# MDIL-SNU/SevenNet

Measured on NVIDIA H100. Metric: atom_updates_per_sec, higher is better.
Workload: dtype f32

## Files before the change

sevenn_b200/csrc/engine.cu:

```cuda
#include <algorithm>
#include <cstdlib>
#include <cstring>
#include <functional>
#include <map>
#include <string>
#include <vector>

#include "../../include/sevenn_b200.h"
#include "common.cuh"
#include "conv_kernels.cuh"
#include "edge_kernels.cuh"
#include "neighbor.cuh"
#include "node_kernels.cuh"
#include "tc_gemm.cuh"

namespace s7b {

static thread_local std::string g_error;
static int64_t g_launches = 0;
extern int64_t g_conv_launches;

void set_error(const char* file, int line, const char* msg) {
  char buf[512];
  snprintf(buf, sizeof(buf), "%s:%d: %s", file, line, msg);
// ... 329 lines not shown
  for (int n = 0; n < N; ++n) {
    double amax = 0.0;
    for (int k = 0; k < K; ++k) amax = std::max(amax, (double)fabsf(W[(size_t)k * N + n]));
    int Eb = 0;
    const bool zero = !(amax > 1e-30);
    if (!zero) frexp(amax, &Eb);
    fb[n] = zero ? 0.0f : (float)ldexp(1.0, Eb - 7);
    const int nt = n / NT, r = n % NT;
    for (int k = 0; k < K; ++k) {
      double sl[3] = {0.0, 0.0, 0.0};
      if (!zero) {
        const double t = ldexp((double)W[(size_t)k * N + n], 23 - Eb);
        const double q0 = nearbyint(t / 65536.0);
        const double r1 = t - q0 * 65536.0;
        const double q1 = nearbyint(r1 / 256.0);
        const double r2 = r1 - q1 * 256.0;
        const double q2 = nearbyint(r2);
        sl[0] = q0; sl[1] = q1 / 256.0; sl[2] = q2 / 65536.0;
      }
      const int kc = k / kTcKC, kk = k % kTcKC;
      const size_t elem = (size_t)((r & 7) * 16 + (r >> 3) * 512 + (kk >> 3) * 128 + (kk & 7) * 2) / 2;
      for (int sidx = 0; sidx < 3; ++sidx)
        q[(((size_t)nt * n_kc + kc) * 3 + sidx) * ((size_t)NT * kTcKC) + elem] = bf16_bits_exact((float)sl[sidx]);
    }
  }
}

static int tc_build_weights(TcWeights& w, const float* host, const int* Ks, const int* Ns, int n_l) {
  w.ok = false;
  w.nblocks = 0;
  size_t q_total = 0, fb_total = 0, woff = 0;
  for (int l = 0; l < n_l; ++l) {
    const int K = Ks[l], N = Ns[l];
    if (K == 0 || N == 0) continue;
    const int NT = tc_pick_nt(N);
    if (NT == 0 || K % kTcKC != 0) return 0;
    TcWeights::Blk& b = w.blk[w.nblocks++];
    b = {K, N, NT, q_total, fb_total};
    q_total += (size_t)3 * K * NT * tc_tiles(N, NT);
    fb_total += (size_t)N;
  }
  std::vector<uint16_t> q(q_total);
  std::vector<float> fb(fb_total);
  int bi = 0;
  for (int l = 0; l < n_l; ++l) {
    const int K = Ks[l], N = Ns[l];
    if (K == 0 || N == 0) continue;
    const TcWeights::Blk& b = w.blk[bi++];
    tc_pack_block(host + woff, K, N, b.NT, q.data() + b.q_off, fb.data() + b.fb_off);
    woff += (size_t)K * N;
  }
  if (w.q.ensure(q_total * sizeof(uint16_t) + 16) || w.fb.ensure(fb_total * sizeof(float) + 16)) return fail("cudaMalloc failed for tensor-core weights");
  S7B_CUDA_CHECK(cudaMemcpy(w.q.p, q.data(), q_total * sizeof(uint16_t), cudaMemcpyHostToDevice));
  S7B_CUDA_CHECK(cudaMemcpy(w.fb.p, fb.data(), fb_total * sizeof(float), cudaMemcpyHostToDevice));
  w.ok = true;
  return 0;
}

typedef CUresult (*EncodeTiledFn)(CUtensorMap*, CUtensorMapDataType, cuuint32_t, void*, const cuuint64_t*, const cuuint64_t*,
                                  const cuuint32_t*, const cuuint32_t*, CUtensorMapInterleave, CUtensorMapSwizzle,
                                  CUtensorMapL2promotion, CUtensorMapFloatOOBfill);
static EncodeTiledFn tensor_map_encoder() {
  static EncodeTiledFn fn = nullptr;
  if (!fn) {
    void* p = nullptr;
    cudaDriverEntryPointQueryResult q;
    if (cudaGetDriverEntryPoint("cuTensorMapEncodeTiled", &p, cudaEnableDefault, &q) == cudaSuccess && q == cudaDriverEntryPointSuccess)
      fn = reinterpret_cast<EncodeTiledFn>(p);
    else cudaGetLastError();
  }
  return fn;
}

static int launch_row_exponents(RowExp& re, const float* A, int lda, const int* a_off, const int* a_K, int n_l,
                                int n_nodes, cudaStream_t st) {
  RowExpArgs r;
  memset(&r, 0, sizeof(r));
  r.A = A;
  r.lda = lda;
  r.n_nodes = n_nodes;
  int rows = 0;
  for (int l = 0; l < n_l; ++l) {
    if (a_K[l] == 0) continue;
    if (a_K[l] % 4 != 0) return fail("row exponents need K % 4 == 0");
    const int b = r.nblocks++;
    r.d[b] = 2 * l + 1;
    r.K[b] = a_K[l];
    r.a_off[b] = a_off[l];
    r.row_base[b] = rows;
    rows += 2 * l + 1;
  }
  r.rows_per_node = rows;
  re.rows_per_node = rows;
  re.bits = false;
  if (rows == 0 || n_nodes == 0) return 0;
  if (re.buf.ensure((size_t)n_nodes * rows * sizeof(int))) return fail("cudaMalloc failed for row exponents");
  r.E = re.buf.as<int>();
  if (rows > 16) return fail("row exponents: more than 16 rows per node");
  const int blk = 256, wpb = blk / 32;
  row_exponent_kernel<<<(n_nodes + wpb - 1) / wpb, blk, 0, st>>>(r);
  S7B_LAUNCH_CHECK();
  return 0;
}

static int launch_tc_linear(const TcWeights& w, const RowExp& re, const float* A, int lda, const int* a_off,
                            const int* a_K, float* C, int ldc, const int* c_off, const int* c_N, int n_l,
                            int n_nodes, bool accumulate, cudaStream_t st) {
  EncodeTiledFn enc = tensor_map_encoder();
  if (!enc) return fail("cuTensorMapEncodeTiled is unavailable (driver too old?)");
  if (ldc % 4 != 0 || (reinterpret_cast<uintptr_t>(C) & 15) != 0) return fail("tensor-core linear: C rows must be 16-byte aligned");
  for (int l = 0; l < n_l; ++l)
    if (c_N[l] != 0 && a_K[l] != 0 && (c_N[l] % 4 != 0 || c_off[l] % 4 != 0)) return fail("tensor-core linear: output blocks must be multiples of 4 floats");
  TcLinArgs t;
  TcMaps maps;
  memset(&t, 0, sizeof(t));
  memset(&maps, 0, sizeof(maps));
  t.C = C;
  t.E = re.buf.as<int>();
  t.ldc = ldc;
  t.n_nodes = n_nodes;
  t.rows_per_node = re.rows_per_node;
  t.accumulate = accumulate ? 1 : 0;
  t.swizzle = g_opt_tc_swizzle;
  t.e_bits = re.bits ? 1 : 0;
  t.trace = g_tc_trace;
  t.trace_cap = g_tc_trace_cap;
  const int n_mt = (n_nodes + kTcBM - 1) / kTcBM;
  int tiles = 0, rows = 0, bi = 0;
  for (int l = 0; l < n_l; ++l) {
    if (a_K[l] == 0 || c_N[l] == 0) { if (a_K[l] != 0) rows += 2 * l + 1; continue; }
    if (bi >= w.nblocks || w.blk[bi].K != a_K[l] || w.blk[bi].N != c_N[l]) return fail("tensor-core weights do not match the call");
    TcLinBlock& b = t.blk[t.nblocks];
    b.Wq = w.q.as<uint16_t>() + w.blk[bi].q_off;
    b.fb = w.fb.as<float>() + w.blk[bi].fb_off;
    b.d = 2 * l + 1;
    b.K = a_K[l];
    b.N = c_N[l];
    b.NT = w.blk[bi].NT;
    b.nnt = tc_tiles(b.N, b.NT);
    b.c_off = c_off[l];
    b.c_cs = c_N[l];
    b.row_base = rows;
    b.tile0 = tiles;
    tiles += n_mt * b.d * b.nnt;
    rows += 2 * l + 1;
    const cuuint64_t gdim[3] = {(cuuint64_t)b.K, (cuuint64_t)b.d, (cuuint64_t)n_nodes};
    const cuuint64_t gstr[2] = {(cuuint64_t)b.K * 4, (cuuint64_t)lda * 4};
    const cuuint32_t box[3] = {(cuuint32_t)kTcKC, 1, (cuuint32_t)kTcBM};
    const cuuint32_t estr[3] = {1, 1, 1};
    const CUresult cr = enc(&maps.m[t.nblocks], CU_TENSOR_MAP_DATA_TYPE_FLOAT32, 3, (void*)(A + a_off[l]), gdim, gstr, box, estr,
                            CU_TENSOR_MAP_INTERLEAVE_NONE, g_opt_tc_swizzle ? CU_TENSOR_MAP_SWIZZLE_128B : CU_TENSOR_MAP_SWIZZLE_NONE,
                            CU_TENSOR_MAP_L2_PROMOTION_L2_128B, CU_TENSOR_MAP_FLOAT_OOB_FILL_NONE);
    if (cr != CUDA_SUCCESS) return fail("cuTensorMapEncodeTiled failed (" + std::to_string((int)cr) + ")");
    ++t.nblocks;
    ++bi;
  }
  if (tiles == 0) return 0;
  t.n_tiles = tiles;
  static int n_sm = 0;
  static bool configured = false;
  if (!configured) {
    int dev = 0;
    S7B_CUDA_CHECK(cudaGetDevice(&dev));
    S7B_CUDA_CHECK(cudaDeviceGetAttribute(&n_sm, cudaDevAttrMultiProcessorCount, dev));
    S7B_CUDA_CHECK(cudaFuncSetAttribute(blocklin_tc_kernel, cudaFuncAttributeMaxDynamicSharedMemorySize, kTcSmemBytes));
    configured = true;
  }
  blocklin_tc_kernel<<<std::min(tiles, n_sm), kTcThreads, kTcSmemBytes, st>>>(t, maps);
  S7B_LAUNCH_CHECK();
  return 0;
}

static int launch_gemm(const LinArgs& a, cudaStream_t st) {
  int max_rows = 0, max_n = 0;
  for (int b = 0; b < a.nblocks; ++b) {
    max_rows = std::max(max_rows, a.n_nodes * a.blk[b].d);
    max_n = std::max(max_n, a.blk[b].N);
  }
  if (max_rows == 0 || max_n == 0) return 0;
  dim3 grid((max_rows + kGemmBM - 1) / kGemmBM, (max_n + kGemmBN - 1) / kGemmBN, a.nblocks);
  blocklin_gemm_kernel<<<grid, kGemmThreads, 0, st>>>(a);
  S7B_LAUNCH_CHECK();
  return 0;
}

static int irreps_linear(const float* A, int lda, const int* a_off, const int* a_K, float* C, int ldc,
                         const int* c_off, const int* c_N, int n_l, const float* W, int n_nodes,
                         bool accumulate, cudaStream_t st) {
  LinArgs a;
  memset(&a, 0, sizeof(a));
  a.A = A;
  a.C = C;
  a.lda = lda;
  a.ldc = ldc;
  a.n_nodes = n_nodes;
  a.accumulate = accumulate ? 1 : 0;
  a.epilogue = kEpiNone;
  a.nblocks = 0;
  size_t woff = 0;
  for (int l = 0; l < n_l; ++l) {
    if (a_K[l] == 0 || c_N[l] == 0) continue;
    LinBlock& b = a.blk[a.nblocks++];
    b.W = W + woff;
    b.d = 2 * l + 1;
    b.K = a_K[l];
    b.N = c_N[l];
    b.a_off = a_off[l];
    b.a_cs = a_K[l];
    b.c_off = c_off[l];
    b.c_cs = c_N[l];
    woff += (size_t)a_K[l] * c_N[l];
  }
  return launch_gemm(a, st);
}

static int node_linear(const LayerCfg& L, const char* name, RowExp& re, bool fresh_re, int n_l_A, const float* A,
                       int lda, const int* a_off, const int* a_K, float* C, int ldc, const int* c_off,
                       const int* c_N, int n_l, const float* W, int n_nodes, bool accumulate, cudaStream_t st) {
  auto it = L.tcw.find(name);
  if (g_opt_tc_gemm && it != L.tcw.end() && it->second && it->second->ok) {
    if (fresh_re && launch_row_exponents(re, A, lda, a_off, a_K, n_l_A, n_nodes, st)) return 1;
    return launch_tc_linear(*it->second, re, A, lda, a_off, a_K, C, ldc, c_off, c_N, n_l, n_nodes, accumulate, st);
  }
  return irreps_linear(A, lda, a_off, a_K, C, ldc, c_off, c_N, n_l, W, n_nodes, accumulate, st);
}

static int dense_gemm(const float* A, int K, float* C, int N, const float* W, int64_t rows, int epilogue,
                      const float* aux_in, float* aux_out, bool accumulate, cudaStream_t st) {
  const int64_t chunk = 1 << 22;
  for (int64_t r0 = 0; r0 < rows; r0 += chunk) {
    const int n = (int)std::min<int64_t>(chunk, rows - r0);
    LinArgs a;
    memset(&a, 0, sizeof(a));
    a.A = A + r0 * K;
    a.C = C + r0 * N;
    a.aux_in = aux_in ? aux_in + r0 * N : nullptr;
    a.aux_out = aux_out ? aux_out + r0 * N : nullptr;
    a.lda = K;
    a.ldc = N;
    a.n_nodes = n;
    a.accumulate = accumulate ? 1 : 0;
    a.epilogue = epilogue;
    a.nblocks = 1;
    a.blk[0] = LinBlock{W, 1, K, N, 0, K, 0, N};
    if (launch_gemm(a, st)) return 1;
  }
  return 0;
}

static int conv_forward(const LayerCfg& L, int lmax_filter, bool table, ConvArgs a, float* out,
                        cudaStream_t st) {
  for (int l1 = 0; l1 < L.n_lx; ++l1)
    if (launch_conv_fwd(l1, lmax_filter, L.lmax_out, table, a, L.roles[l1], out, st)) return 1;
  return 0;
}

}

extern "C" {

const char* s7b_last_error(void) { return g_error.c_str(); }
int s7b_version(void) { return 1; }
int64_t s7b_launch_count(int reset) {
  const int64_t v = g_launches + g_conv_launches;
  if (reset) { g_launches = 0; g_conv_launches = 0; }
  return v;
}

int s7b_set_option(const char* name, int value) {
  if (!name) return fail("null option name");
  if (std::string(name) == "tc_gemm") { g_opt_tc_gemm = value; return 0; }
  if (std::string(name) == "tc_swizzle") { g_opt_tc_swizzle = value; return 0; }
  if (std::string(name) == "atomic_virial") { g_opt_atomic_virial = value; return 0; }
  if (std::string(name) == "concurrent_conv") { g_opt_concurrent = value; return 0; }
  if (std::string(name) == "cuda_graph") { g_opt_cuda_graph = value; return 0; }
  if (std::string(name) == "stage_graphs") { g_opt_stage_graphs = value; return 0; }
  if (std::string(name) == "gate_bwd_rows") { g_opt_gate_bwd_rows = value; return 0; }
  return fail(std::string("unknown option: ") + name);
}

int s7b_gather_rows(const float* src, int32_t ld_src, const int32_t* idx, int64_t n, int32_t width, float* out, void* stream) {
  if (n <= 0 || width <= 0) return 0;
  cudaStream_t st = reinterpret_cast<cudaStream_t>(stream);
  const bool vec = width % 4 == 0 && ld_src % 4 == 0 && (reinterpret_cast<uintptr_t>(src) | reinterpret_cast<uintptr_t>(out)) % 16 == 0;
  const size_t total = (size_t)n * (vec ? width / 4 : width);
  const int grd = (int)std::min<size_t>((total + 255) / 256, 132 * 16);
  if (vec) gather_rows_idx_kernel<true><<<grd, 256, 0, st>>>(src, ld_src, idx, n, width, out);
  else gather_rows_idx_kernel<false><<<grd, 256, 0, st>>>(src, ld_src, idx, n, width, out);
  S7B_LAUNCH_CHECK();
  return 0;
}

int s7b_scatter_add_rows(float* dst, int32_t ld_dst, const int32_t* idx, int64_t n, int32_t width, const float* in, void* stream) {
  if (n <= 0 || width <= 0) return 0;
  cudaStream_t st = reinterpret_cast<cudaStream_t>(stream);
  const bool vec = width % 4 == 0 && ld_dst % 4 == 0 && (reinterpret_cast<uintptr_t>(dst) | reinterpret_cast<uintptr_t>(in)) % 16 == 0;
  const size_t total = (size_t)n * (vec ? width / 4 : width);
  const int grd = (int)std::min<size_t>((total + 255) / 256, 132 * 16);
  if (vec) scatter_add_rows_idx_kernel<true><<<grd, 256, 0, st>>>(dst, ld_dst, idx, n, width, in);
  else scatter_add_rows_idx_kernel<false><<<grd, 256, 0, st>>>(dst, ld_dst, idx, n, width, in);
  S7B_LAUNCH_CHECK();
  return 0;
}

int s7b_dense_linear(const float* A, const float* W, float* C, int64_t rows, int32_t K, int32_t N,
                     int32_t use_tc, void* stream) {
// ... 1158 lines not shown
```

sevenn_b200/csrc/tc_gemm.cuh:

```cuda
#pragma once
#include <cuda.h>
#include <cuda_bf16.h>

#include <type_traits>

#include "common.cuh"
#include "node_kernels.cuh"

namespace s7b {

constexpr int kTcBM = 64;
constexpr int kTcKC = 32;
constexpr int kTcMaxNT = 128;
constexpr int kTcAccRegs = kTcMaxNT / 2;
constexpr int kTcThreads = 320;
constexpr int kTcXformThreads = 128;
constexpr int kTcMmaWarps = 4;
constexpr int kTcRawBytes = kTcBM * kTcKC * 4;
constexpr int kTcASliceBytes = kTcBM * kTcKC * 2;
constexpr int kTcBSliceBytes = kTcMaxNT * kTcKC * 2;
constexpr int kTcRawStages = 8, kTcOpsStages = 3, kTcWStages = 3;
constexpr int kTcOpsBytes = 3 * kTcASliceBytes, kTcWBytes = 3 * kTcBSliceBytes;
constexpr int kTcRawOff = 0;
constexpr int kTcOpsOff = kTcRawOff + kTcRawStages * kTcRawBytes;
constexpr int kTcWOff = kTcOpsOff + kTcOpsStages * kTcOpsBytes;
constexpr int kTcSmemBytes = kTcWOff + kTcWStages * kTcWBytes + 1024 ;
constexpr int kTcZeroRow = -1000;

__device__ __forceinline__ uint32_t smem_u32(const void* p) {
  return static_cast<uint32_t>(__cvta_generic_to_shared(p));
}
__device__ __forceinline__ void mbar_init(uint64_t* bar, uint32_t count) {
  asm volatile("mbarrier.init.shared::cta.b64 [%0], %1;" ::"r"(smem_u32(bar)), "r"(count) : "memory");
}
__device__ __forceinline__ void mbar_wait(uint64_t* bar, uint32_t parity) {
  asm volatile(
      "{\n"
      ".reg .pred P1;\n"
      "LAB_WAIT:\n"
      "mbarrier.try_wait.parity.shared::cta.b64 P1, [%0], %1;\n"
      "@P1 bra DONE;\n"
      "bra LAB_WAIT;\n"
      "DONE:\n"
      "}\n" ::"r"(smem_u32(bar)), "r"(parity) : "memory");
}
__device__ __forceinline__ void mbar_arrive(uint64_t* bar) {
  asm volatile("mbarrier.arrive.shared::cta.b64 _, [%0];" ::"r"(smem_u32(bar)) : "memory");
}
__device__ __forceinline__ void mbar_arrive_after(uint64_t* bar, float dep) {
  asm volatile(
      "{\n"
      ".reg .pred p;\n"
      "setp.ne.b32 p, %1, 0x7fc12345;\n"
      "@p mbarrier.arrive.shared::cta.b64 _, [%0];\n"
      "}\n" ::"r"(smem_u32(bar)), "r"(__float_as_uint(dep)) : "memory");
}
__device__ __forceinline__ void mbar_expect_tx(uint64_t* bar, uint32_t bytes) {
  asm volatile("mbarrier.arrive.expect_tx.shared::cta.b64 _, [%0], %1;" ::"r"(smem_u32(bar)), "r"(bytes) : "memory");
}
__device__ __forceinline__ void fence_async_smem() { asm volatile("fence.proxy.async.shared::cta;" ::: "memory"); }

__device__ __forceinline__ void tma_load_3d(void* dst, const CUtensorMap* map, int c0, int c1, int c2, uint64_t* bar) {
  asm volatile(
      "cp.async.bulk.tensor.3d.shared::cluster.global.tile.mbarrier::complete_tx::bytes [%0], [%1, {%2, %3, %4}], [%5];"
      ::"r"(smem_u32(dst)), "l"(reinterpret_cast<uint64_t>(map)), "r"(c0), "r"(c1), "r"(c2), "r"(smem_u32(bar))
      : "memory");
}
__device__ __forceinline__ void bulk_load(void* dst, const void* src, uint32_t bytes, uint64_t* bar) {
  asm volatile(
      "cp.async.bulk.shared::cluster.global.mbarrier::complete_tx::bytes [%0], [%1], %2, [%3];"
      ::"r"(smem_u32(dst)), "l"(reinterpret_cast<uint64_t>(src)), "r"(bytes), "r"(smem_u32(bar))
      : "memory");
}

__device__ __forceinline__ uint64_t gmma_desc(uint32_t saddr) {
  return (uint64_t)((saddr & 0x3FFFF) >> 4) | ((uint64_t)(128 >> 4) << 16) | ((uint64_t)(512 >> 4) << 32);
}
__device__ __forceinline__ void wgmma_fence() { asm volatile("wgmma.fence.sync.aligned;" ::: "memory"); }
__device__ __forceinline__ void wgmma_commit() { asm volatile("wgmma.commit_group.sync.aligned;" ::: "memory"); }
template <int N>
__device__ __forceinline__ void wgmma_wait() { asm volatile("wgmma.wait_group.sync.aligned %0;" ::"n"(N) : "memory"); }
__device__ __forceinline__ void acc_fence(float (&d)[kTcAccRegs]) {
#pragma unroll
  for (int i = 0; i < kTcAccRegs; ++i) asm volatile("" : "+f"(d[i])::"memory");
}
template <int N>
__device__ __forceinline__ void wgmma_bf16(float (&d)[kTcAccRegs], uint64_t da, uint64_t db, uint32_t scale_d);
template <> __device__ __forceinline__ void wgmma_bf16<16>(float (&d)[kTcAccRegs], uint64_t da, uint64_t db, uint32_t scale_d) {
  asm volatile(
      "{\n.reg .pred p;\nsetp.ne.b32 p, %10, 0;\n"
      "wgmma.mma_async.sync.aligned.m64n16k16.f32.bf16.bf16 {%0, %1, %2, %3, %4, %5, %6, %7}, %8, %9, p, 1, 1, 0, 0;\n}\n"
      : "+f"(d[0]), "+f"(d[1]), "+f"(d[2]), "+f"(d[3]), "+f"(d[4]), "+f"(d[5]), "+f"(d[6]), "+f"(d[7])
      : "l"(da), "l"(db), "r"(scale_d));
}
template <> __device__ __forceinline__ void wgmma_bf16<32>(float (&d)[kTcAccRegs], uint64_t da, uint64_t db, uint32_t scale_d) {
  asm volatile(
      "{\n.reg .pred p;\nsetp.ne.b32 p, %18, 0;\n"
      "wgmma.mma_async.sync.aligned.m64n32k16.f32.bf16.bf16 {%0, %1, %2, %3, %4, %5, %6, %7, %8, %9, %10, %11, %12, %13, %14, %15}, %16, %17, p, 1, 1, 0, 0;\n}\n"
      : "+f"(d[0]), "+f"(d[1]), "+f"(d[2]), "+f"(d[3]), "+f"(d[4]), "+f"(d[5]), "+f"(d[6]), "+f"(d[7]), "+f"(d[8]), "+f"(d[9]), "+f"(d[10]), "+f"(d[11]), "+f"(d[12]), "+f"(d[13]), "+f"(d[14]), "+f"(d[15])
      : "l"(da), "l"(db), "r"(scale_d));
}
template <> __device__ __forceinline__ void wgmma_bf16<48>(float (&d)[kTcAccRegs], uint64_t da, uint64_t db, uint32_t scale_d) {
  asm volatile(
      "{\n.reg .pred p;\nsetp.ne.b32 p, %26, 0;\n"
      "wgmma.mma_async.sync.aligned.m64n48k16.f32.bf16.bf16 {%0, %1, %2, %3, %4, %5, %6, %7, %8, %9, %10, %11, %12, %13, %14, %15, %16, %17, %18, %19, %20, %21, %22, %23}, %24, %25, p, 1, 1, 0, 0;\n}\n"
      : "+f"(d[0]), "+f"(d[1]), "+f"(d[2]), "+f"(d[3]), "+f"(d[4]), "+f"(d[5]), "+f"(d[6]), "+f"(d[7]), "+f"(d[8]), "+f"(d[9]), "+f"(d[10]), "+f"(d[11]), "+f"(d[12]), "+f"(d[13]), "+f"(d[14]), "+f"(d[15]), "+f"(d[16]), "+f"(d[17]), "+f"(d[18]), "+f"(d[19]), "+f"(d[20]), "+f"(d[21]), "+f"(d[22]), "+f"(d[23])
      : "l"(da), "l"(db), "r"(scale_d));
}
template <> __device__ __forceinline__ void wgmma_bf16<64>(float (&d)[kTcAccRegs], uint64_t da, uint64_t db, uint32_t scale_d) {
  asm volatile(
      "{\n.reg .pred p;\nsetp.ne.b32 p, %34, 0;\n"
      "wgmma.mma_async.sync.aligned.m64n64k16.f32.bf16.bf16 {%0, %1, %2, %3, %4, %5, %6, %7, %8, %9, %10, %11, %12, %13, %14, %15, %16, %17, %18, %19, %20, %21, %22, %23, %24, %25, %26, %27, %28, %29, %30, %31}, %32, %33, p, 1, 1, 0, 0;\n}\n"
      : "+f"(d[0]), "+f"(d[1]), "+f"(d[2]), "+f"(d[3]), "+f"(d[4]), "+f"(d[5]), "+f"(d[6]), "+f"(d[7]), "+f"(d[8]), "+f"(d[9]), "+f"(d[10]), "+f"(d[11]), "+f"(d[12]), "+f"(d[13]), "+f"(d[14]), "+f"(d[15]), "+f"(d[16]), "+f"(d[17]), "+f"(d[18]), "+f"(d[19]), "+f"(d[20]), "+f"(d[21]), "+f"(d[22]), "+f"(d[23]), "+f"(d[24]), "+f"(d[25]), "+f"(d[26]), "+f"(d[27]), "+f"(d[28]), "+f"(d[29]), "+f"(d[30]), "+f"(d[31])
      : "l"(da), "l"(db), "r"(scale_d));
}
template <> __device__ __forceinline__ void wgmma_bf16<80>(float (&d)[kTcAccRegs], uint64_t da, uint64_t db, uint32_t scale_d) {
  asm volatile(
      "{\n.reg .pred p;\nsetp.ne.b32 p, %42, 0;\n"
      "wgmma.mma_async.sync.aligned.m64n80k16.f32.bf16.bf16 {%0, %1, %2, %3, %4, %5, %6, %7, %8, %9, %10, %11, %12, %13, %14, %15, %16, %17, %18, %19, %20, %21, %22, %23, %24, %25, %26, %27, %28, %29, %30, %31, %32, %33, %34, %35, %36, %37, %38, %39}, %40, %41, p, 1, 1, 0, 0;\n}\n"
      : "+f"(d[0]), "+f"(d[1]), "+f"(d[2]), "+f"(d[3]), "+f"(d[4]), "+f"(d[5]), "+f"(d[6]), "+f"(d[7]), "+f"(d[8]), "+f"(d[9]), "+f"(d[10]), "+f"(d[11]), "+f"(d[12]), "+f"(d[13]), "+f"(d[14]), "+f"(d[15]), "+f"(d[16]), "+f"(d[17]), "+f"(d[18]), "+f"(d[19]), "+f"(d[20]), "+f"(d[21]), "+f"(d[22]), "+f"(d[23]), "+f"(d[24]), "+f"(d[25]), "+f"(d[26]), "+f"(d[27]), "+f"(d[28]), "+f"(d[29]), "+f"(d[30]), "+f"(d[31]), "+f"(d[32]), "+f"(d[33]), "+f"(d[34]), "+f"(d[35]), "+f"(d[36]), "+f"(d[37]), "+f"(d[38]), "+f"(d[39])
      : "l"(da), "l"(db), "r"(scale_d));
}
template <> __device__ __forceinline__ void wgmma_bf16<96>(float (&d)[kTcAccRegs], uint64_t da, uint64_t db, uint32_t scale_d) {
  asm volatile(
      "{\n.reg .pred p;\nsetp.ne.b32 p, %50, 0;\n"
      "wgmma.mma_async.sync.aligned.m64n96k16.f32.bf16.bf16 {%0, %1, %2, %3, %4, %5, %6, %7, %8, %9, %10, %11, %12, %13, %14, %15, %16, %17, %18, %19, %20, %21, %22, %23, %24, %25, %26, %27, %28, %29, %30, %31, %32, %33, %34, %35, %36, %37, %38, %39, %40, %41, %42, %43, %44, %45, %46, %47}, %48, %49, p, 1, 1, 0, 0;\n}\n"
      : "+f"(d[0]), "+f"(d[1]), "+f"(d[2]), "+f"(d[3]), "+f"(d[4]), "+f"(d[5]), "+f"(d[6]), "+f"(d[7]), "+f"(d[8]), "+f"(d[9]), "+f"(d[10]), "+f"(d[11]), "+f"(d[12]), "+f"(d[13]), "+f"(d[14]), "+f"(d[15]), "+f"(d[16]), "+f"(d[17]), "+f"(d[18]), "+f"(d[19]), "+f"(d[20]), "+f"(d[21]), "+f"(d[22]), "+f"(d[23]), "+f"(d[24]), "+f"(d[25]), "+f"(d[26]), "+f"(d[27]), "+f"(d[28]), "+f"(d[29]), "+f"(d[30]), "+f"(d[31]), "+f"(d[32]), "+f"(d[33]), "+f"(d[34]), "+f"(d[35]), "+f"(d[36]), "+f"(d[37]), "+f"(d[38]), "+f"(d[39]), "+f"(d[40]), "+f"(d[41]), "+f"(d[42]), "+f"(d[43]), "+f"(d[44]), "+f"(d[45]), "+f"(d[46]), "+f"(d[47])
      : "l"(da), "l"(db), "r"(scale_d));
}
template <> __device__ __forceinline__ void wgmma_bf16<112>(float (&d)[kTcAccRegs], uint64_t da, uint64_t db, uint32_t scale_d) {
  asm volatile(
      "{\n.reg .pred p;\nsetp.ne.b32 p, %58, 0;\n"
      "wgmma.mma_async.sync.aligned.m64n112k16.f32.bf16.bf16 {%0, %1, %2, %3, %4, %5, %6, %7, %8, %9, %10, %11, %12, %13, %14, %15, %16, %17, %18, %19, %20, %21, %22, %23, %24, %25, %26, %27, %28, %29, %30, %31, %32, %33, %34, %35, %36, %37, %38, %39, %40, %41, %42, %43, %44, %45, %46, %47, %48, %49, %50, %51, %52, %53, %54, %55}, %56, %57, p, 1, 1, 0, 0;\n}\n"
      : "+f"(d[0]), "+f"(d[1]), "+f"(d[2]), "+f"(d[3]), "+f"(d[4]), "+f"(d[5]), "+f"(d[6]), "+f"(d[7]), "+f"(d[8]), "+f"(d[9]), "+f"(d[10]), "+f"(d[11]), "+f"(d[12]), "+f"(d[13]), "+f"(d[14]), "+f"(d[15]), "+f"(d[16]), "+f"(d[17]), "+f"(d[18]), "+f"(d[19]), "+f"(d[20]), "+f"(d[21]), "+f"(d[22]), "+f"(d[23]), "+f"(d[24]), "+f"(d[25]), "+f"(d[26]), "+f"(d[27]), "+f"(d[28]), "+f"(d[29]), "+f"(d[30]), "+f"(d[31]), "+f"(d[32]), "+f"(d[33]), "+f"(d[34]), "+f"(d[35]), "+f"(d[36]), "+f"(d[37]), "+f"(d[38]), "+f"(d[39]), "+f"(d[40]), "+f"(d[41]), "+f"(d[42]), "+f"(d[43]), "+f"(d[44]), "+f"(d[45]), "+f"(d[46]), "+f"(d[47]), "+f"(d[48]), "+f"(d[49]), "+f"(d[50]), "+f"(d[51]), "+f"(d[52]), "+f"(d[53]), "+f"(d[54]), "+f"(d[55])
      : "l"(da), "l"(db), "r"(scale_d));
}
template <> __device__ __forceinline__ void wgmma_bf16<128>(float (&d)[kTcAccRegs], uint64_t da, uint64_t db, uint32_t scale_d) {
  asm volatile(
      "{\n.reg .pred p;\nsetp.ne.b32 p, %66, 0;\n"
      "wgmma.mma_async.sync.aligned.m64n128k16.f32.bf16.bf16 {%0, %1, %2, %3, %4, %5, %6, %7, %8, %9, %10, %11, %12, %13, %14, %15, %16, %17, %18, %19, %20, %21, %22, %23, %24, %25, %26, %27, %28, %29, %30, %31, %32, %33, %34, %35, %36, %37, %38, %39, %40, %41, %42, %43, %44, %45, %46, %47, %48, %49, %50, %51, %52, %53, %54, %55, %56, %57, %58, %59, %60, %61, %62, %63}, %64, %65, p, 1, 1, 0, 0;\n}\n"
      : "+f"(d[0]), "+f"(d[1]), "+f"(d[2]), "+f"(d[3]), "+f"(d[4]), "+f"(d[5]), "+f"(d[6]), "+f"(d[7]), "+f"(d[8]), "+f"(d[9]), "+f"(d[10]), "+f"(d[11]), "+f"(d[12]), "+f"(d[13]), "+f"(d[14]), "+f"(d[15]), "+f"(d[16]), "+f"(d[17]), "+f"(d[18]), "+f"(d[19]), "+f"(d[20]), "+f"(d[21]), "+f"(d[22]), "+f"(d[23]), "+f"(d[24]), "+f"(d[25]), "+f"(d[26]), "+f"(d[27]), "+f"(d[28]), "+f"(d[29]), "+f"(d[30]), "+f"(d[31]), "+f"(d[32]), "+f"(d[33]), "+f"(d[34]), "+f"(d[35]), "+f"(d[36]), "+f"(d[37]), "+f"(d[38]), "+f"(d[39]), "+f"(d[40]), "+f"(d[41]), "+f"(d[42]), "+f"(d[43]), "+f"(d[44]), "+f"(d[45]), "+f"(d[46]), "+f"(d[47]), "+f"(d[48]), "+f"(d[49]), "+f"(d[50]), "+f"(d[51]), "+f"(d[52]), "+f"(d[53]), "+f"(d[54]), "+f"(d[55]), "+f"(d[56]), "+f"(d[57]), "+f"(d[58]), "+f"(d[59]), "+f"(d[60]), "+f"(d[61]), "+f"(d[62]), "+f"(d[63])
      : "l"(da), "l"(db), "r"(scale_d));
}

__device__ __forceinline__ float exp2i(int e) {
  e = e < -126 ? -126 : (e > 127 ? 127 : e);
  return __int_as_float((e + 127) << 23);
}

struct RowExpArgs {
  const float* A;
  int* E;
  int lda, n_nodes, rows_per_node, nblocks;
  int d[kMaxL], K[kMaxL], a_off[kMaxL], row_base[kMaxL];
};

__global__ void row_exponent_kernel(const RowExpArgs a) {
  __shared__ unsigned int smax[8][16];
  const int wib = threadIdx.x >> 5, lane = threadIdx.x & 31;
  const int n = blockIdx.x * (blockDim.x >> 5) + wib;
  if (lane < 16) smax[wib][lane] = 0u;
  __syncwarp();
  if (n < a.n_nodes) {
    for (int b = 0; b < a.nblocks; ++b) {
      const int K = a.K[b], quads = (a.d[b] * K) >> 2;
      const float4* row = reinterpret_cast<const float4*>(a.A + (size_t)n * a.lda + a.a_off[b]);
      for (int q0 = 0; q0 < quads; q0 += 32) {
        const int q = q0 + lane;
        unsigned int m = 0u;
        int r = -1;
        if (q < quads) {
          const float4 v = __ldg(row + q);
          m = __float_as_uint(v.x) & 0x7fffffffu;
          m = max(m, __float_as_uint(v.y) & 0x7fffffffu);
          m = max(m, __float_as_uint(v.z) & 0x7fffffffu);
          m = max(m, __float_as_uint(v.w) & 0x7fffffffu);
          r = a.row_base[b] + (4 * q) / K;
        }
        const unsigned int peers = __match_any_sync(0xffffffffu, r);
        const unsigned int mm = __reduce_max_sync(peers, m);
        if (r >= 0 && lane == __ffs(peers) - 1) smax[wib][r] = max(smax[wib][r], mm);
        __syncwarp();
      }
    }
  }
  __syncwarp();
  if (n < a.n_nodes && lane < a.rows_per_node) {
    const int ex = (int)(smax[wib][lane] >> 23);
    a.E[(size_t)n * a.rows_per_node + lane] = (ex == 0 || ex == 255) ? kTcZeroRow : max(ex - 126, -104);
  }
}

struct TcLinBlock {
  const uint16_t* Wq;
  const float* fb;
  int d, K, N, NT, nnt;
  int c_off, c_cs;
  int row_base;
  int tile0;
};
struct TcLinArgs {
  float* C;
  const int* E;
  int ldc, n_nodes, rows_per_node, accumulate, nblocks, n_tiles, swizzle;
  int e_bits;
  long long* trace;
  int trace_cap;
  TcLinBlock blk[kMaxL];
};
#define TC_TRACE(role, ev, idx)                                                                   \
  do {                                                                                            \
    if (a.trace != nullptr && blockIdx.x == 0) {                                                  \
      const int per = a.trace_cap / 5;                                                            \
      if (trace_n < per) {                                                                        \
        long long* rec = a.trace + 8 + 3 * ((size_t)(role) * per + trace_n);                      \
        rec[0] = (ev);                                                                            \
        rec[1] = (long long)(idx);                                                                \
        rec[2] = clock64();                                                                       \
        ++trace_n;                                                                                \
        a.trace[1 + (role)] = trace_n;                                                            \
      }                                                                                           \
    }                                                                                             \
  } while (0)
struct TcMaps { CUtensorMap m[kMaxL]; };

__device__ __forceinline__ float4 lds128(uint32_t saddr) {
  float4 v;
  asm volatile("ld.shared.v4.f32 {%0, %1, %2, %3}, [%4];" : "=f"(v.x), "=f"(v.y), "=f"(v.z), "=f"(v.w) : "r"(saddr) : "memory");
  return v;
}
__device__ __forceinline__ void sts128(uint32_t saddr, uint32_t a, uint32_t b, uint32_t c, uint32_t d) {
  asm volatile("st.shared.v4.b32 [%0], {%1, %2, %3, %4};" ::"r"(saddr), "r"(a), "r"(b), "r"(c), "r"(d) : "memory");
}

__device__ __forceinline__ uint32_t pack_bf16(float lo, float hi) {
  const __nv_bfloat162 v = __floats2bfloat162_rn(lo, hi);
  return *reinterpret_cast<const uint32_t*>(&v);
}

template <int N>
__device__ __forceinline__ void tc_mma_chunk(float (&acc0)[kTcAccRegs], float (&acc1)[kTcAccRegs], uint32_t sa,
                                             uint32_t sb, bool first) {
  constexpr uint32_t b_slice = (uint32_t)N * kTcKC * 2u;
#pragma unroll
  for (int j = 0; j < kTcKC / 16; ++j) {
    const uint32_t ko = (uint32_t)j * 256u;
    const uint64_t dA0 = gmma_desc(sa + ko);
    const uint64_t dA1 = gmma_desc(sa + kTcASliceBytes + ko);
    const uint64_t dA2 = gmma_desc(sa + 2 * kTcASliceBytes + ko);
    const uint64_t dB0 = gmma_desc(sb + ko);
    const uint64_t dB1 = gmma_desc(sb + b_slice + ko);
    const uint64_t dB2 = gmma_desc(sb + 2 * b_slice + ko);
    const uint32_t acc = (!first || j > 0) ? 1u : 0u;
    wgmma_bf16<N>(acc0, dA0, dB0, acc);
    wgmma_bf16<N>(acc1, dA0, dB1, acc);
    wgmma_bf16<N>(acc1, dA1, dB0, 1u);
    wgmma_bf16<N>(acc1, dA0, dB2, 1u);
    wgmma_bf16<N>(acc1, dA1, dB1, 1u);
    wgmma_bf16<N>(acc1, dA2, dB0, 1u);
  }
}

__global__ void __launch_bounds__(kTcThreads, 1)
blocklin_tc_kernel(const TcLinArgs a, const __grid_constant__ TcMaps maps) {
  extern __shared__ uint8_t smem_raw[];
  uint8_t* smem = reinterpret_cast<uint8_t*>((reinterpret_cast<uintptr_t>(smem_raw) + 1023) & ~(uintptr_t)1023);
  __shared__ uint64_t bar_raw_full[kTcRawStages], bar_raw_empty[kTcRawStages];
  __shared__ uint64_t bar_ops_full[kTcOpsStages], bar_ops_empty[kTcOpsStages];
  __shared__ uint64_t bar_w_full[kTcWStages], bar_w_empty[kTcWStages];

  const int tid = threadIdx.x, warp = tid >> 5, lane = tid & 31;
  int trace_n = 0;

  if (tid == 0) {
    for (int s = 0; s < kTcRawStages; ++s) { mbar_init(&bar_raw_full[s], 1); mbar_init(&bar_raw_empty[s], kTcXformThreads); }
    for (int s = 0; s < kTcOpsStages; ++s) { mbar_init(&bar_ops_full[s], kTcXformThreads); mbar_init(&bar_ops_empty[s], kTcMmaWarps); }
    for (int s = 0; s < kTcWStages; ++s) { mbar_init(&bar_w_full[s], 1); mbar_init(&bar_w_empty[s], kTcMmaWarps); }
    asm volatile("fence.mbarrier_init.release.cluster;" ::: "memory");
  }
  __syncthreads();

  auto decode = [&](int t, int& b, int& mt, int& ci, int& nt) {
    b = 0;
    while (b + 1 < a.nblocks && t >= a.blk[b + 1].tile0) ++b;
    const int rel = t - a.blk[b].tile0;
    const int nnt = a.blk[b].nnt;
    nt = rel % nnt;
    const int r2 = rel / nnt;
    ci = r2 % a.blk[b].d;
    mt = r2 / a.blk[b].d;
  };
  auto row_exp = [&](int t, int row) -> int {
    if (t >= a.n_tiles) return kTcZeroRow;
    int b, mt, ci, nt;
    decode(t, b, mt, ci, nt);
    const int node = mt * kTcBM + row;
    if (node >= a.n_nodes) return kTcZeroRow;
    int v = __ldg(a.E + (size_t)node * a.rows_per_node + a.blk[b].row_base + ci);
    if (a.e_bits) {
      const int ex = v >> 23;
      v = (ex == 0 || ex == 255) ? kTcZeroRow : max(ex - 126, -104);
    }
    return v;
  };

  if (warp == 8) {
    if (lane == 0) {
      uint32_t it = 0;
      for (int t = blockIdx.x; t < a.n_tiles; t += gridDim.x) {
        int b, mt, ci, nt;
        decode(t, b, mt, ci, nt);
        const int n_kc = a.blk[b].K / kTcKC;
        for (int kc = 0; kc < n_kc; ++kc, ++it) {
          const int s = it % kTcRawStages;
          mbar_wait(&bar_raw_empty[s], ((it / kTcRawStages) & 1) ^ 1);
          TC_TRACE(0, 0, it);
          mbar_expect_tx(&bar_raw_full[s], (uint32_t)kTcRawBytes);
          tma_load_3d(smem + kTcRawOff + (size_t)s * kTcRawBytes, &maps.m[b], kc * kTcKC, ci, mt * kTcBM, &bar_raw_full[s]);
        }
      }
    }
  } else if (warp == 9) {
    if (lane == 0) {
      uint32_t it = 0;
      for (int t = blockIdx.x; t < a.n_tiles; t += gridDim.x) {
        int b, mt, ci, nt;
        decode(t, b, mt, ci, nt);
        const TcLinBlock& B = a.blk[b];
        const int n_kc = B.K / kTcKC;
        const uint32_t b_bytes = 3u * (uint32_t)B.NT * kTcKC * 2u;
        const uint8_t* wsrc = reinterpret_cast<const uint8_t*>(B.Wq) + (size_t)nt * n_kc * b_bytes;
        for (int kc = 0; kc < n_kc; ++kc, ++it) {
          const int s = it % kTcWStages;
          mbar_wait(&bar_w_empty[s], ((it / kTcWStages) & 1) ^ 1);
          TC_TRACE(4, 0, it);
          mbar_expect_tx(&bar_w_full[s], b_bytes);
          bulk_load(smem + kTcWOff + (size_t)s * kTcWBytes, wsrc + (size_t)kc * b_bytes, b_bytes, &bar_w_full[s]);
        }
      }
    }
  } else if (warp < 4) {
    const int r = tid & (kTcBM - 1), h = tid / kTcBM;
    const uint32_t swz = a.swizzle ? (uint32_t)(r & 7) : 0u;
    const uint32_t row_off = (uint32_t)((r & 7) * 16 + (r >> 3) * 512);
    const V2 M2 = splat2(12582912.0f), nM2 = splat2(-12582912.0f);
    uint32_t it = 0;
    int Ea_next = row_exp(blockIdx.x, r);
    for (int t = blockIdx.x; t < a.n_tiles; t += gridDim.x) {
      int b, mt, ci, nt;
      decode(t, b, mt, ci, nt);
      const int n_kc = a.blk[b].K / kTcKC;
      const int Ea = Ea_next;
      Ea_next = row_exp(t + gridDim.x, r);
      const float sc = (Ea == kTcZeroRow) ? 0.0f : exp2i(23 - Ea);
      for (int kc = 0; kc < n_kc; ++kc, ++it) {
        const int s = it % kTcRawStages, o = it % kTcOpsStages;
        mbar_wait(&bar_raw_full[s], (it / kTcRawStages) & 1);
        if (tid == 0) TC_TRACE(1, 0, it);
        const uint32_t raw = smem_u32(smem + kTcRawOff + (size_t)s * kTcRawBytes + (size_t)r * 128);
        float4 v[4];
#pragma unroll
        for (int q = 0; q < 4; ++q) v[q] = lds128(raw + (((uint32_t)(4 * h + q) ^ swz) << 4));
        const float dep = (v[0].x + v[1].x) + (v[2].x + v[3].x);
        mbar_arrive_after(&bar_raw_empty[s], dep);
        mbar_wait(&bar_ops_empty[o], ((it / kTcOpsStages) & 1) ^ 1);
        if (tid == 0) TC_TRACE(1, 1, it);
        const uint32_t a0 = smem_u32(smem + kTcOpsOff + (size_t)o * kTcOpsBytes);
        const uint32_t a1 = a0 + kTcASliceBytes, a2 = a1 + kTcASliceBytes;
#pragma unroll
        for (int kk = 0; kk < 2; ++kk) {
          const V2 x[4] = {make_float2(v[2 * kk].x, v[2 * kk].y), make_float2(v[2 * kk].z, v[2 * kk].w),
                           make_float2(v[2 * kk + 1].x, v[2 * kk + 1].y), make_float2(v[2 * kk + 1].z, v[2 * kk + 1].w)};
          uint32_t p0[4], p1[4], p2[4];
#pragma unroll
          for (int j = 0; j < 4; ++j) {
            const V2 tt = mul_(x[j], sc);
            const V2 q0 = add_(fma_(tt, splat2(1.52587890625e-05f), M2), nM2);
            const V2 r1 = fma_(q0, splat2(-65536.0f), tt);
            const V2 q1 = add_(fma_(r1, splat2(0.00390625f), M2), nM2);
            const V2 r2 = fma_(q1, splat2(-256.0f), r1);
            const V2 q2 = add_(add_(r2, M2), nM2);
            const V2 s1 = mul_(q1, 0.00390625f), s2 = mul_(q2, 1.52587890625e-05f);
            p0[j] = pack_bf16(q0.x, q0.y);
            p1[j] = pack_bf16(s1.x, s1.y);
            p2[j] = pack_bf16(s2.x, s2.y);
          }
          const uint32_t off = row_off + (uint32_t)(2 * h + kk) * 128u;
          sts128(a0 + off, p0[0], p0[1], p0[2], p0[3]);
          sts128(a1 + off, p1[0], p1[1], p1[2], p1[3]);
          sts128(a2 + off, p2[0], p2[1], p2[2], p2[3]);
        }
        fence_async_smem();
        if (tid == 0) TC_TRACE(1, 2, it);
        mbar_arrive(&bar_ops_full[o]);
      }
    }
  } else if (warp < 8) {
    const int mw = warp - 4, q4 = lane & 3;
    const int rl = 16 * mw + (lane >> 2);
    float acc0[kTcAccRegs], acc1[kTcAccRegs];
#pragma unroll
    for (int i = 0; i < kTcAccRegs; ++i) { acc0[i] = 0.0f; acc1[i] = 0.0f; }
    uint32_t it = 0, tile_it = 0;
    int Ea_next0 = row_exp(blockIdx.x, rl), Ea_next1 = row_exp(blockIdx.x, rl + 8);
    for (int t = blockIdx.x; t < a.n_tiles; t += gridDim.x, ++tile_it) {
      int b, mt, ci, nt;
      decode(t, b, mt, ci, nt);
      const TcLinBlock& B = a.blk[b];
      const int n_kc = B.K / kTcKC;
      const int Ea0 = Ea_next0, Ea1 = Ea_next1;
      Ea_next0 = row_exp(t + gridDim.x, rl);
      Ea_next1 = row_exp(t + gridDim.x, rl + 8);
      auto mainloop = [&](auto width) {
        constexpr int N = decltype(width)::value;
        int prev_o = 0, prev_w = 0;
        for (int kc = 0; kc < n_kc; ++kc, ++it) {
          const int o = it % kTcOpsStages, w = it % kTcWStages;
          mbar_wait(&bar_w_full[w], (it / kTcWStages) & 1);
          if (tid == 128) TC_TRACE(2, 0, it);
          mbar_wait(&bar_ops_full[o], (it / kTcOpsStages) & 1);
          if (tid == 128) TC_TRACE(2, 1, it);
          __syncwarp();
          const uint32_t sa = smem_u32(smem + kTcOpsOff + (size_t)o * kTcOpsBytes);
          const uint32_t sb = smem_u32(smem + kTcWOff + (size_t)w * kTcWBytes);
          acc_fence(acc0);
          acc_fence(acc1);
          wgmma_fence();
          tc_mma_chunk<N>(acc0, acc1, sa, sb, kc == 0);
          wgmma_commit();
          acc_fence(acc0);
          acc_fence(acc1);
          wgmma_wait<1>();
          if (kc > 0) {
            __syncwarp();
            if (lane == 0) { mbar_arrive(&bar_ops_empty[prev_o]); mbar_arrive(&bar_w_empty[prev_w]); }
          }
          prev_o = o;
          prev_w = w;
        }
        wgmma_wait<0>();
        acc_fence(acc0);
        acc_fence(acc1);
        __syncwarp();
        if (lane == 0) { mbar_arrive(&bar_ops_empty[prev_o]); mbar_arrive(&bar_w_empty[prev_w]); }
      };
      switch (B.NT) {
        case 16: mainloop(std::integral_constant<int, 16>()); break;
        case 32: mainloop(std::integral_constant<int, 32>()); break;
        case 48: mainloop(std::integral_constant<int, 48>()); break;
        case 64: mainloop(std::integral_constant<int, 64>()); break;
        case 80: mainloop(std::integral_constant<int, 80>()); break;
        case 96: mainloop(std::integral_constant<int, 96>()); break;
        case 112: mainloop(std::integral_constant<int, 112>()); break;
        default: mainloop(std::integral_constant<int, 128>()); break;
      }
      if (tid == 160) TC_TRACE(3, 0, tile_it);

      const float fa0 = (Ea0 == kTcZeroRow) ? 0.0f : exp2i(Ea0 - 7);
      const float fa1 = (Ea1 == kTcZeroRow) ? 0.0f : exp2i(Ea1 - 7);
      const int col0 = nt * B.NT;
      const int node0 = mt * kTcBM + rl;
      const bool ok0 = node0 < a.n_nodes, ok1 = node0 + 8 < a.n_nodes;
      float* c0 = a.C + (size_t)node0 * a.ldc + B.c_off + (size_t)ci * B.c_cs + col0 + 2 * q4;
      float* c1 = c0 + (size_t)8 * a.ldc;
      const float* fbp = B.fb + col0 + 2 * q4;
#pragma unroll
      for (int j = 0; j < kTcMaxNT / 8; ++j) {
        if (8 * j < B.NT && col0 + 8 * j + 2 * q4 < B.N) {
          const float2 fb2 = __ldg(reinterpret_cast<const float2*>(fbp + 8 * j));
          const float2 v0 = make_float2((acc0[4 * j + 0] + acc1[4 * j + 0]) * fa0 * fb2.x,
                                        (acc0[4 * j + 1] + acc1[4 * j + 1]) * fa0 * fb2.y);
          const float2 v1 = make_float2((acc0[4 * j + 2] + acc1[4 * j + 2]) * fa1 * fb2.x,
                                        (acc0[4 * j + 3] + acc1[4 * j + 3]) * fa1 * fb2.y);
          if (a.accumulate) {
            if (ok0) atomicAdd(reinterpret_cast<float2*>(c0 + 8 * j), v0);
            if (ok1) atomicAdd(reinterpret_cast<float2*>(c1 + 8 * j), v1);
          } else {
            if (ok0) *reinterpret_cast<float2*>(c0 + 8 * j) = v0;
            if (ok1) *reinterpret_cast<float2*>(c1 + 8 * j) = v1;
          }
        }
      }
      if (tid == 160) TC_TRACE(3, 1, tile_it);
    }
  }
}

}
```

Before: 1.537 million.

## Stage GEMM epilogue in swizzled shared memory and write C via TMA store/reduce

Replaces the per-thread float2 global stores and atomicAdds in the tensor-core linear kernel epilogue with a swizzled shared-memory staging tile that one thread writes out using TMA bulk tensor stores or reduce-add. A C tensor map per block is encoded on the host, and the fb scale vector is staged in shared memory. To make room for the 32KB C staging buffer, raw stages drop from 8 to 4 and weight stages rise from 3 to 5. This adds a named barrier across the MMA warps and a wait on the previous bulk store before reusing the buffer, which can serialize the epilogue with the next tile's mainloop.

```diff
diff --git a/sevenn_b200/csrc/engine.cu b/sevenn_b200/csrc/engine.cu
--- a/sevenn_b200/csrc/engine.cu
+++ b/sevenn_b200/csrc/engine.cu
@@ -505,6 +505,13 @@
                             CU_TENSOR_MAP_INTERLEAVE_NONE, g_opt_tc_swizzle ? CU_TENSOR_MAP_SWIZZLE_128B : CU_TENSOR_MAP_SWIZZLE_NONE,
                             CU_TENSOR_MAP_L2_PROMOTION_L2_128B, CU_TENSOR_MAP_FLOAT_OOB_FILL_NONE);
     if (cr != CUDA_SUCCESS) return fail("cuTensorMapEncodeTiled failed (" + std::to_string((int)cr) + ")");
+    const cuuint64_t cdim[3] = {(cuuint64_t)b.N, (cuuint64_t)b.d, (cuuint64_t)n_nodes};
+    const cuuint64_t cstr[2] = {(cuuint64_t)b.c_cs * 4, (cuuint64_t)ldc * 4};
+    const cuuint32_t cbox[3] = {(cuuint32_t)kTcCBox, 1, (cuuint32_t)kTcBM};
+    const CUresult cc = enc(&maps.c[t.nblocks], CU_TENSOR_MAP_DATA_TYPE_FLOAT32, 3, (void*)(C + c_off[l]), cdim, cstr, cbox, estr,
+                            CU_TENSOR_MAP_INTERLEAVE_NONE, CU_TENSOR_MAP_SWIZZLE_64B, CU_TENSOR_MAP_L2_PROMOTION_NONE,
+                            CU_TENSOR_MAP_FLOAT_OOB_FILL_NONE);
+    if (cc != CUDA_SUCCESS) return fail("cuTensorMapEncodeTiled failed for C (" + std::to_string((int)cc) + ")");
     ++t.nblocks;
     ++bi;
   }
diff --git a/sevenn_b200/csrc/tc_gemm.cuh b/sevenn_b200/csrc/tc_gemm.cuh
--- a/sevenn_b200/csrc/tc_gemm.cuh
+++ b/sevenn_b200/csrc/tc_gemm.cuh
@@ -19,12 +19,17 @@
 constexpr int kTcRawBytes = kTcBM * kTcKC * 4;
 constexpr int kTcASliceBytes = kTcBM * kTcKC * 2;
 constexpr int kTcBSliceBytes = kTcMaxNT * kTcKC * 2;
-constexpr int kTcRawStages = 8, kTcOpsStages = 3, kTcWStages = 3;
+constexpr int kTcRawStages = 4, kTcOpsStages = 3, kTcWStages = 5;
 constexpr int kTcOpsBytes = 3 * kTcASliceBytes, kTcWBytes = 3 * kTcBSliceBytes;
+constexpr int kTcCBox = 16;
+constexpr int kTcCBoxBytes = kTcBM * kTcCBox * 4;
+constexpr int kTcCBytes = kTcBM * kTcMaxNT * 4;
 constexpr int kTcRawOff = 0;
 constexpr int kTcOpsOff = kTcRawOff + kTcRawStages * kTcRawBytes;
 constexpr int kTcWOff = kTcOpsOff + kTcOpsStages * kTcOpsBytes;
-constexpr int kTcSmemBytes = kTcWOff + kTcWStages * kTcWBytes + 1024 ;
+constexpr int kTcCOff = kTcWOff + kTcWStages * kTcWBytes;
+constexpr int kTcSmemBytes = kTcCOff + kTcCBytes + 1024 ;
+static_assert(kTcCOff % 1024 == 0, "the swizzled C staging tile must be 1024-byte aligned");
 constexpr int kTcZeroRow = -1000;
 
 __device__ __forceinline__ uint32_t smem_u32(const void* p) {
@@ -71,6 +76,21 @@
       "cp.async.bulk.shared::cluster.global.mbarrier::complete_tx::bytes [%0], [%1], %2, [%3];"
       ::"r"(smem_u32(dst)), "l"(reinterpret_cast<uint64_t>(src)), "r"(bytes), "r"(smem_u32(bar))
       : "memory");
+}
+__device__ __forceinline__ void tma_store_3d(const CUtensorMap* map, uint32_t src, int c0, int c1, int c2) {
+  asm volatile("cp.async.bulk.tensor.3d.global.shared::cta.tile.bulk_group [%0, {%1, %2, %3}], [%4];"
+               ::"l"(reinterpret_cast<uint64_t>(map)), "r"(c0), "r"(c1), "r"(c2), "r"(src) : "memory");
+}
+__device__ __forceinline__ void tma_reduce_add_3d(const CUtensorMap* map, uint32_t src, int c0, int c1, int c2) {
+  asm volatile("cp.reduce.async.bulk.tensor.3d.global.shared::cta.add.tile.bulk_group [%0, {%1, %2, %3}], [%4];"
+               ::"l"(reinterpret_cast<uint64_t>(map)), "r"(c0), "r"(c1), "r"(c2), "r"(src) : "memory");
+}
+__device__ __forceinline__ void bulk_commit() { asm volatile("cp.async.bulk.commit_group;" ::: "memory"); }
+__device__ __forceinline__ void bulk_wait_read_all() { asm volatile("cp.async.bulk.wait_group.read 0;" ::: "memory"); }
+__device__ __forceinline__ void bulk_wait_all() { asm volatile("cp.async.bulk.wait_group 0;" ::: "memory"); }
+__device__ __forceinline__ void mma_group_sync() { asm volatile("bar.sync 1, 128;" ::: "memory"); }
+__device__ __forceinline__ void sts64(uint32_t saddr, float x, float y) {
+  asm volatile("st.shared.v2.f32 [%0], {%1, %2};" ::"r"(saddr), "f"(x), "f"(y) : "memory");
 }
 
 __device__ __forceinline__ uint64_t gmma_desc(uint32_t saddr) {
@@ -222,7 +242,7 @@
       }                                                                                           \
     }                                                                                             \
   } while (0)
-struct TcMaps { CUtensorMap m[kMaxL]; };
+struct TcMaps { CUtensorMap m[kMaxL], c[kMaxL]; };
 
 __device__ __forceinline__ float4 lds128(uint32_t saddr) {
   float4 v;
@@ -268,6 +288,7 @@
   __shared__ uint64_t bar_raw_full[kTcRawStages], bar_raw_empty[kTcRawStages];
   __shared__ uint64_t bar_ops_full[kTcOpsStages], bar_ops_empty[kTcOpsStages];
   __shared__ uint64_t bar_w_full[kTcWStages], bar_w_empty[kTcWStages];
+  __shared__ __align__(16) float fb_s[kTcMaxNT];
 
   const int tid = threadIdx.x, warp = tid >> 5, lane = tid & 31;
   int trace_n = 0;
@@ -396,8 +417,13 @@
       }
     }
   } else if (warp < 8) {
-    const int mw = warp - 4, q4 = lane & 3;
+    const int mw = warp - 4, q4 = lane & 3, ct = tid - 128;
     const int rl = 16 * mw + (lane >> 2);
+    const uint32_t cst = smem_u32(smem + kTcCOff);
+    auto c_addr = [&](int r, int j) -> uint32_t {
+      const int g = 2 * (j & 1) + (q4 >> 1);
+      return cst + (uint32_t)((j >> 1) * kTcCBoxBytes + r * 64 + ((g ^ ((r >> 1) & 3)) << 4) + (q4 & 1) * 8);
+    };
     float acc0[kTcAccRegs], acc1[kTcAccRegs];
 #pragma unroll
     for (int i = 0; i < kTcAccRegs; ++i) { acc0[i] = 0.0f; acc1[i] = 0.0f; }
@@ -411,7 +437,9 @@
       const int Ea0 = Ea_next0, Ea1 = Ea_next1;
       Ea_next0 = row_exp(t + gridDim.x, rl);
       Ea_next1 = row_exp(t + gridDim.x, rl + 8);
-      auto mainloop = [&](auto width) {
+      const int col0 = nt * B.NT;
+      const float fb_t = (ct < B.NT && col0 + ct < B.N) ? __ldg(B.fb + col0 + ct) : 0.0f;
+      auto run_tile = [&](auto width) {
         constexpr int N = decltype(width)::value;
         int prev_o = 0, prev_w = 0;
         for (int kc = 0; kc < n_kc; ++kc, ++it) {
@@ -443,46 +471,47 @@
         acc_fence(acc1);
         __syncwarp();
         if (lane == 0) { mbar_arrive(&bar_ops_empty[prev_o]); mbar_arrive(&bar_w_empty[prev_w]); }
+        if (tid == 160) TC_TRACE(3, 0, tile_it);
+
+        const float fa0 = (Ea0 == kTcZeroRow) ? 0.0f : exp2i(Ea0 - 7);
+        const float fa1 = (Ea1 == kTcZeroRow) ? 0.0f : exp2i(Ea1 - 7);
+        if (tid == 128) bulk_wait_read_all();
+        fb_s[ct] = fb_t;
+        mma_group_sync();
+        if (tid == 160) TC_TRACE(3, 2, tile_it);
+#pragma unroll
+        for (int j = 0; j < N / 8; ++j) {
+          const float2 fb2 = *reinterpret_cast<const float2*>(&fb_s[8 * j + 2 * q4]);
+          sts64(c_addr(rl, j), (acc0[4 * j + 0] + acc1[4 * j + 0]) * fa0 * fb2.x,
+                (acc0[4 * j + 1] + acc1[4 * j + 1]) * fa0 * fb2.y);
+          sts64(c_addr(rl + 8, j), (acc0[4 * j + 2] + acc1[4 * j + 2]) * fa1 * fb2.x,
+                (acc0[4 * j + 3] + acc1[4 * j + 3]) * fa1 * fb2.y);
+        }
+        if (tid == 160) TC_TRACE(3, 3, tile_it);
       };
       switch (B.NT) {
-        case 16: mainloop(std::integral_constant<int, 16>()); break;
-        case 32: mainloop(std::integral_constant<int, 32>()); break;
-        case 48: mainloop(std::integral_constant<int, 48>()); break;
-        case 64: mainloop(std::integral_constant<int, 64>()); break;
-        case 80: mainloop(std::integral_constant<int, 80>()); break;
-        case 96: mainloop(std::integral_constant<int, 96>()); break;
-        case 112: mainloop(std::integral_constant<int, 112>()); break;
-        default: mainloop(std::integral_constant<int, 128>()); break;
+        case 16: run_tile(std::integral_constant<int, 16>()); break;
+        case 32: run_tile(std::integral_constant<int, 32>()); break;
+        case 48: run_tile(std::integral_constant<int, 48>()); break;
+        case 64: run_tile(std::integral_constant<int, 64>()); break;
+        case 80: run_tile(std::integral_constant<int, 80>()); break;
+        case 96: run_tile(std::integral_constant<int, 96>()); break;
+        case 112: run_tile(std::integral_constant<int, 112>()); break;
+        default: run_tile(std::integral_constant<int, 128>()); break;
       }
-      if (tid == 160) TC_TRACE(3, 0, tile_it);
-
-      const float fa0 = (Ea0 == kTcZeroRow) ? 0.0f : exp2i(Ea0 - 7);
-      const float fa1 = (Ea1 == kTcZeroRow) ? 0.0f : exp2i(Ea1 - 7);
-      const int col0 = nt * B.NT;
-      const int node0 = mt * kTcBM + rl;
-      const bool ok0 = node0 < a.n_nodes, ok1 = node0 + 8 < a.n_nodes;
-      float* c0 = a.C + (size_t)node0 * a.ldc + B.c_off + (size_t)ci * B.c_cs + col0 + 2 * q4;
-      float* c1 = c0 + (size_t)8 * a.ldc;
-      const float* fbp = B.fb + col0 + 2 * q4;
-#pragma unroll
-      for (int j = 0; j < kTcMaxNT / 8; ++j) {
-        if (8 * j < B.NT && col0 + 8 * j + 2 * q4 < B.N) {
-          const float2 fb2 = __ldg(reinterpret_cast<const float2*>(fbp + 8 * j));
-          const float2 v0 = make_float2((acc0[4 * j + 0] + acc1[4 * j + 0]) * fa0 * fb2.x,
-                                        (acc0[4 * j + 1] + acc1[4 * j + 1]) * fa0 * fb2.y);
-          const float2 v1 = make_float2((acc0[4 * j + 2] + acc1[4 * j + 2]) * fa1 * fb2.x,
-                                        (acc0[4 * j + 3] + acc1[4 * j + 3]) * fa1 * fb2.y);
-          if (a.accumulate) {
-            if (ok0) atomicAdd(reinterpret_cast<float2*>(c0 + 8 * j), v0);
-            if (ok1) atomicAdd(reinterpret_cast<float2*>(c1 + 8 * j), v1);
-          } else {
-            if (ok0) *reinterpret_cast<float2*>(c0 + 8 * j) = v0;
-            if (ok1) *reinterpret_cast<float2*>(c1 + 8 * j) = v1;
-          }
-        }
+      fence_async_smem();
+      mma_group_sync();
+      if (tid == 128) {
+        for (int s = 0; s < B.NT / kTcCBox && col0 + s * kTcCBox < B.N; ++s) {
+          const uint32_t src = cst + (uint32_t)(s * kTcCBoxBytes);
+          if (a.accumulate) tma_reduce_add_3d(&maps.c[b], src, col0 + s * kTcCBox, ci, mt * kTcBM);
+          else tma_store_3d(&maps.c[b], src, col0 + s * kTcCBox, ci, mt * kTcBM);
+        }
+        bulk_commit();
       }
       if (tid == 160) TC_TRACE(3, 1, tile_it);
     }
+    if (tid == 128) bulk_wait_all();
   }
 }
 
```

Result: faster. 1.611 million (median of 6 runs) (+4.9%).
